# thunlp/ConvDR

Measured on AMD Instinct MI355X. Metric: passages encoded/sec + query x passage IP-scored/sec, 768-d, higher is better.
Workload: dtype bf16

## Files before the change

convdr_amd/csrc/encoder.hip:

```cpp
#include "gemm_launch.hpp"
#include "gemm_ln.hpp"
#include "cls_fold.hpp"

#include "../../include/convdr_hip.h"

namespace convdr {

struct EncBufs {
  int32_t* status;
  int32_t *tok_id, *tok_pos;
  bf16_t *X, *Q, *K, *Vt, *ctx, *Hm, *cls_b, *cls_ctx, *cls_x, *cls_x1;
  float *Y, *cls_y, *cls_f, *head_y;
  float* slab;
  int64_t ldt;
  size_t total;
};

constexpr int64_t SPLITK_MAX_ROWS = 42 * 128;
constexpr int SPLITK_MAX_SPLIT = 4;
static int64_t g_ffn2_splitk = 1;

static EncBufs enc_plan(const convdr_encoder_config* c, int64_t rows, int B, char* base) {
  EncBufs p;
  size_t o = 0;
// ... 226 lines not shown
}

extern "C" int convdr_encoder_forward(const convdr_encoder_config* cfg, const convdr_encoder_weights* w,
                                      const void* input_ids, int ids_are_int32, const int64_t* attention_mask, int B, int L,
                                      const int32_t* cu_seqlens, const int32_t* seq_lens, int64_t rows, int max_len,
                                      void* workspace, size_t workspace_bytes, float* out, convdr_stream_t stream) {
  hipStream_t st = (hipStream_t)stream;
  if (int e = check_config(cfg)) return e;
  CONVDR_REQUIRE(B > 0 && L > 0 && rows > 0 && rows % 8 == 0 && max_len > 0 && max_len <= L,
                 "convdr_encoder_forward: bad sizes B=%d L=%d rows=%lld max_len=%d", B, L, (long long)rows, max_len);
  const EncBufs p = enc_plan(cfg, rows, B, (char*)workspace);
  CONVDR_REQUIRE(workspace_bytes >= p.total, "convdr_encoder_forward: workspace too small (%zu < %zu)", workspace_bytes,
                 p.total);
  const int H = cfg->hidden;
  CONVDR_CHECK_HIP(hipMemset2DAsync(p.Vt + rows, p.ldt * 2, 0, (p.ldt - rows) * 2, H, st));
  CONVDR_CHECK_HIP(hipMemsetAsync(p.status, 0, 256, st));
  hipLaunchKernelGGL(k_seq_pack, dim3((B + 3) / 4), dim3(256), 0, st, input_ids, ids_are_int32, attention_mask, seq_lens, B, L, cu_seqlens,
                     cfg->kind, cfg->pad_idx, cfg->max_pos, cfg->vocab, p.tok_id, p.tok_pos, p.status);
  CONVDR_CHECK_LAUNCH("k_seq_pack");
  return encoder_forward_packed(cfg, w, p, cu_seqlens, seq_lens, rows, B, max_len, out, st);
}

extern "C" int convdr_encoder_forward_ragged(const convdr_encoder_config* cfg, const convdr_encoder_weights* w,
                                             const int32_t* tokens, int64_t n_tokens, const int32_t* tok_offsets, int B,
                                             const int32_t* cu_seqlens, const int32_t* seq_lens, int64_t rows, int max_len,
                                             void* workspace, size_t workspace_bytes, float* out, convdr_stream_t stream) {
  hipStream_t st = (hipStream_t)stream;
  if (int e = check_config(cfg)) return e;
  CONVDR_REQUIRE(B > 0 && n_tokens >= B && n_tokens <= INT32_MAX && rows > 0 && rows % 8 == 0 && rows >= n_tokens && max_len > 0 &&
                     max_len <= n_tokens,
                 "convdr_encoder_forward_ragged: bad sizes B=%d n_tokens=%lld rows=%lld max_len=%d", B, (long long)n_tokens,
                 (long long)rows, max_len);
  CONVDR_REQUIRE(tokens != nullptr && tok_offsets != nullptr, "convdr_encoder_forward_ragged: null tokens / tok_offsets");
  const EncBufs p = enc_plan(cfg, rows, B, (char*)workspace);
  CONVDR_REQUIRE(workspace_bytes >= p.total, "convdr_encoder_forward_ragged: workspace too small (%zu < %zu)", workspace_bytes,
                 p.total);
  const int H = cfg->hidden;
  CONVDR_CHECK_HIP(hipMemset2DAsync(p.Vt + rows, p.ldt * 2, 0, (p.ldt - rows) * 2, H, st));
  CONVDR_CHECK_HIP(hipMemsetAsync(p.status, 0, 256, st));
  hipLaunchKernelGGL(k_seq_pack_ragged, dim3((B + 3) / 4), dim3(256), 0, st, tokens, n_tokens, tok_offsets, seq_lens, B, cu_seqlens,
                     cfg->kind, cfg->pad_idx, cfg->max_pos, cfg->vocab, p.tok_id, p.tok_pos, p.status);
  CONVDR_CHECK_LAUNCH("k_seq_pack_ragged");
  return encoder_forward_packed(cfg, w, p, cu_seqlens, seq_lens, rows, B, max_len, out, st);
}

extern "C" int convdr_encoder_debug_layout(const convdr_encoder_config* cfg, int64_t rows, int B, int64_t* out) {
  const EncBufs p = enc_plan(cfg, rows, B, nullptr);
  const void* v[13] = {p.tok_id, p.tok_pos, p.X, p.Q, p.K, p.Vt, p.ctx, p.Hm, p.Y, p.cls_b, p.cls_y, p.cls_f, p.head_y};
  for (int i = 0; i < 13; ++i) out[i] = (int64_t)(size_t)v[i];
  out[13] = p.ldt;
  return 0;
}

namespace convdr {
static __global__ void __launch_bounds__(256) k_pack_kslice(const bf16_t* __restrict__ w, int n, int k, bf16_t* __restrict__ out) {
  const int64_t total = (int64_t)n * (k / 8);
  for (int64_t i = (int64_t)blockIdx.x * blockDim.x + threadIdx.x; i < total; i += (int64_t)gridDim.x * blockDim.x) {
    const int c = (int)(i & 3);
    const int64_t sr = i >> 2;
    const int r = (int)(sr % n), s = (int)(sr / n);
    *(uint4*)(out + i * 8) = *(const uint4*)(w + (int64_t)r * k + s * 32 + c * 8);
  }
}
}

extern "C" int convdr_pack_kslice(const void* w_bf16, int n, int k, void* out, convdr_stream_t stream) {
  CONVDR_REQUIRE(n > 0 && k > 0 && k % 32 == 0, "convdr_pack_kslice: bad shape %d x %d", n, k);
  const int64_t total = (int64_t)n * (k / 8);
  hipLaunchKernelGGL(k_pack_kslice, dim3((unsigned)(ceil_div64(total, 256) < 4096 ? ceil_div64(total, 256) : 4096)), dim3(256), 0,
                     (hipStream_t)stream, (const bf16_t*)w_bf16, n, k, (bf16_t*)out);
  CONVDR_CHECK_LAUNCH("k_pack_kslice");
  return 0;
}

extern "C" int convdr_set_option(const char* name, int64_t value) {
  if (strcmp(name, "fused_ln_min_rows") == 0) {
    g_fused_ln_min_rows = value;
    return 0;
  }
  if (strcmp(name, "hm_blocked") == 0) {
    g_hm_blocked = value;
    return 0;
  }
  if (strcmp(name, "cls_fold") == 0) {
    g_cls_fold = value;
    return 0;
  }
  if (strcmp(name, "cls_fold_min_rows") == 0) {
    g_cls_fold_min_rows = value;
    return 0;
  }
  if (strcmp(name, "gemm_tile_policy") == 0) {
    g_gemm_tile_policy = value;
    return 0;
  }
  if (strcmp(name, "attn_bwd_fused") == 0) {
    g_attn_bwd_fused = value;
    return 0;
  }
  if (strcmp(name, "embed_bwd_deterministic") == 0) {
    g_embed_bwd_det = value;
    return 0;
  }
  if (strcmp(name, "ip_fused_finish") == 0) {
    convdr::g_ip_fused_finish = value;
    return 0;
  }
  if (strcmp(name, "gelu_gp") == 0) {
    g_gelu_gp = value;
    return 0;
  }
  if (strcmp(name, "ffn2_splitk") == 0) {
    g_ffn2_splitk = value;
    return 0;
  }
  if (strcmp(name, "ln_rows") == 0) {
    g_ln_rows = value;
    return 0;
  }
  if (strcmp(name, "ln_bwd_rows") == 0) {
    g_ln_bwd_rows = value;
    return 0;
  }
  if (strcmp(name, "train_bwd_stop_layer") == 0) {
    g_train_bwd_stop_layer = value;
    return 0;
  }
  if (strcmp(name, "fused_ln_max_k") == 0) {
    g_fused_ln_max_k = value;
    return 0;
  }
  if (strcmp(name, "clock_probe") == 0) {
    g_clock_probe = (void*)(uintptr_t)value;
    g_clock_probe_next = 0;
    return 0;
  }
  if (strcmp(name, "clock_probe_slots") == 0) {
    g_clock_probe_slots = value > 0 ? value : 1;
    return 0;
  }
  if (strcmp(name, "attn_trace") == 0) {
    g_attn_trace = (void*)(uintptr_t)value;
    return 0;
  }
  if (strcmp(name, "gemm_trace_ln") == 0) {
    g_gemm_trace_ln = (void*)(uintptr_t)value;
    return 0;
  }
  if (strcmp(name, "gemm_trace") == 0) {
    g_gemm_trace = (void*)(uintptr_t)value;
    return 0;
  }
  set_error("convdr_set_option: unknown option %s", name);
  return -1;
}
```

convdr_amd/csrc/encoder_kernels.hpp:

```cpp
#pragma once
#include "../../include/convdr_hip.h"
#include "dropout.hpp"
#include "gemm_nt.hpp"

namespace convdr {

static __global__ void __launch_bounds__(256) k_seq_pack(const void* __restrict__ ids_v, int ids32,
                                                  const int64_t* __restrict__ mask, const int32_t* __restrict__ lens,
                                                  int B, int L, const int32_t* __restrict__ cu, int kind, int pad_idx,
                                                  int max_pos, int vocab, int32_t* __restrict__ tok_id,
                                                  int32_t* __restrict__ tok_pos, int32_t* __restrict__ status) {
  const int lane = threadIdx.x & 63;
  const int b = blockIdx.x * 4 + (threadIdx.x >> 6);
  if (b >= B) return;
  const int base = cu[b], end = cu[b + 1];
  const int64_t* ids = (const int64_t*)ids_v;
  const int32_t* ids_i = (const int32_t*)ids_v;
  const int len_b = lens[b];
  int kept = 0, nonpad = 0;
  int flags = 0;
  for (int l0 = 0; l0 < L; l0 += 64) {
    const int l = l0 + lane;
    const bool valid = l < L;
    int64_t id = valid ? (ids32 ? (int64_t)ids_i[(int64_t)b * L + l] : ids[(int64_t)b * L + l]) : (int64_t)pad_idx;
    const bool m = valid && (mask ? mask[(int64_t)b * L + l] != 0 : l < len_b);
    if (l == 0 && !m) flags |= CONVDR_ENC_STATUS_BAD_MASK;
    const bool np = valid && id != pad_idx;
    const unsigned long long bm = __ballot(m), bnp = __ballot(np);
    const unsigned long long lt = (1ull << lane) - 1ull;
    if (m) {
      if (id < 0 || id >= (int64_t)vocab) { flags |= CONVDR_ENC_STATUS_BAD_TOKEN; id = 0; }
      const int row = base + kept + __popcll(bm & lt);
      if (row < end) {
        int p = kind == 0 ? (np ? nonpad + __popcll(bnp & (lt | (1ull << lane))) + pad_idx : pad_idx) : l;
        p = p < max_pos ? p : max_pos - 1;
        tok_id[row] = (int)id;
        tok_pos[row] = p;
      }
    }
    kept += __popcll(bm);
    nonpad += __popcll(bnp);
  }
  if (kept != len_b) flags |= CONVDR_ENC_STATUS_BAD_LENS;
  if (__ballot(flags != 0) != 0ull) {
#pragma unroll
    for (int o = 32; o >= 1; o >>= 1) flags |= __shfl_xor(flags, o, 64);
    if (lane == 0) atomicOr(status, flags);
  }
  for (int r = base + kept + lane; r < end; r += 64) {
    tok_id[r] = -1;
    tok_pos[r] = 0;
  }
}

static __global__ void __launch_bounds__(256) k_seq_pack_ragged(const int32_t* __restrict__ tokens, int64_t n_tokens,
                                                         const int32_t* __restrict__ off, const int32_t* __restrict__ lens,
                                                         int B, const int32_t* __restrict__ cu, int kind, int pad_idx,
                                                         int max_pos, int vocab, int32_t* __restrict__ tok_id,
                                                         int32_t* __restrict__ tok_pos, int32_t* __restrict__ status) {
  const int lane = threadIdx.x & 63;
  const int b = blockIdx.x * 4 + (threadIdx.x >> 6);
  if (b >= B) return;
  const int base = cu[b], end = cu[b + 1];
  const int64_t o0 = off[b], o1 = off[b + 1];
  const int len_b = lens[b];
  const bool ok = o0 >= 0 && o0 <= o1 && o1 <= n_tokens && o1 - o0 == (int64_t)len_b && len_b >= 1 &&
                  (int64_t)len_b <= (int64_t)end - (int64_t)base;
  const int n = ok ? len_b : 0;
  int kept = 0, nonpad = 0;
  int flags = ok ? 0 : CONVDR_ENC_STATUS_BAD_LENS;
  for (int l0 = 0; l0 < n; l0 += 64) {
    const int l = l0 + lane;
    const bool m = l < n;
    int id = m ? tokens[o0 + l] : pad_idx;
    const bool np = m && id != pad_idx;
    const unsigned long long bm = __ballot(m), bnp = __ballot(np);
    const unsigned long long lt = (1ull << lane) - 1ull;
    if (m) {
      if (id < 0 || id >= vocab) { flags |= CONVDR_ENC_STATUS_BAD_TOKEN; id = 0; }
      const int row = base + kept + __popcll(bm & lt);
      int p = kind == 0 ? (np ? nonpad + __popcll(bnp & (lt | (1ull << lane))) + pad_idx : pad_idx) : l;
      p = p < max_pos ? p : max_pos - 1;
      tok_id[row] = id;
// ... 372 lines not shown
struct CTile {
  static constexpr int PASSES = (T::TL * T::TR * 2) / T::STAGE_BYTES;
  static constexpr int NTP = T::NT / PASSES;
  static constexpr int ROWS = T::TL / PASSES;
  static_assert(PASSES >= 1 && PASSES * NTP == T::NT, "a pass is a whole number of MFMA column blocks");
  static constexpr int HALF = ROWS / 2, HALF_BYTES = HALF * T::TR * 2;
  struct Base { uint32_t lo, hi; };
  __device__ static __forceinline__ Base contiguous(const char* sC) {
    static_assert(2 * HALF_BYTES <= T::STAGE_BYTES, "a parked pass must fit the idle stage");
    return Base{lds_off(sC), lds_off(sC) + HALF_BYTES};
  }
  static constexpr int CW = T::MT * 4;
  static constexpr int RW = NTP * 32;
  static constexpr int W_BYTES = RW * CW * 16;
  static constexpr int W_STORES = RW * CW / 64;
  static_assert(W_BYTES * T::WAVES <= 2 * HALF_BYTES && (64 % CW) == 0, "wave-local park must fit the pass image");
  __device__ static __forceinline__ uint32_t wave_base(Base sC, int wave) {
    constexpr int PER_HALF = HALF_BYTES / W_BYTES;
    return (wave >= PER_HALF ? sC.hi + (wave - PER_HALF) * W_BYTES : sC.lo + wave * W_BYTES);
  }
  __device__ static __forceinline__ void put_w(uint32_t wb, const WavePos<T>& w, int mt, int ntl, int g, uint2 o) {
    const int row = ntl * 32 + w.li;
    lds_write_b64_hidden(wb + row * (CW * 16) + (((mt * 4 + g) ^ (row & (CW - 1))) << 4) + w.hi * 8, (u32x2_t){o.x, o.y});
  }
  template <int C0, int CN>
  __device__ static __forceinline__ void store_w_part(bool nt, uint32_t wb, int lane, bf16_t* dst, int64_t ld, int64_t row_limit,
                                                      int64_t col_limit) {
    constexpr int RPI = 64 / CN, N_ST = RW / RPI;
    static_assert(64 % CN == 0 && N_ST % 4 == 0, "store_w_part geometry");
    const int r0 = lane / CN, c = C0 + (lane - r0 * CN);
    const int64_t nv = col_limit - c * 8;
#pragma unroll
    for (int i0 = 0; i0 < N_ST; i0 += 4) {
      u32x4_t v[4];
      auto at = [&](int i) {
        const int row = i * RPI + r0;
        return wb + row * (CW * 16) + ((c ^ (row & (CW - 1))) << 4);
      };
      lds_read4_b128_hidden(at(i0), at(i0 + 1), at(i0 + 2), at(i0 + 3), v[0], v[1], v[2], v[3]);
#pragma unroll
      for (int j = 0; j < 4; ++j) {
        const int row = (i0 + j) * RPI + r0;
        bf16_t* pr = dst + (int64_t)row * ld + c * 8;
        if (row < row_limit && nv > 0) {
          if (nv >= 8) {
            if (nt) store16<true>(pr, v[j]);
            else store16<false>(pr, v[j]);
          }
          else *(uint2*)pr = make_uint2(v[j].x, v[j].y);
        }
      }
    }
  }
  __device__ static __forceinline__ void store_w(bool nt, uint32_t wb, int lane, bf16_t* dst, int64_t ld, int64_t row_limit,
                                                 int64_t col_limit) {
    constexpr int RPI = 64 / CW;
    const int r0 = lane / CW, c = lane - r0 * CW;
    const int64_t nv = col_limit - c * 8;
    static_assert(W_STORES % 4 == 0, "lds_read4_b128_hidden reads four chunks");
#pragma unroll
    for (int i0 = 0; i0 < W_STORES; i0 += 4) {
      u32x4_t v[4];
      auto at = [&](int i) {
        const int row = i * RPI + r0;
        return wb + row * (CW * 16) + ((c ^ (row & (CW - 1))) << 4);
      };
      lds_read4_b128_hidden(at(i0), at(i0 + 1), at(i0 + 2), at(i0 + 3), v[0], v[1], v[2], v[3]);
#pragma unroll
      for (int j = 0; j < 4; ++j) {
        const int row = (i0 + j) * RPI + r0;
        bf16_t* pr = dst + (int64_t)row * ld + c * 8;
        if (row < row_limit && nv > 0) {
          if (nv >= 8) {
            if (nt) store16<true>(pr, v[j]);
            else store16<false>(pr, v[j]);
          }
          else *(uint2*)pr = make_uint2(v[j].x, v[j].y);
        }
      }
    }
  }
};

template <int EPI, class T>
static __global__ void __launch_bounds__(T::THREADS, 2) k_gemm(const GemmArgs a) {
  extern __shared__ __attribute__((aligned(16))) char smem[];
  using CT = CTile<T>;
  const WavePos<T> w;
  const int64_t ldw = a.ldw ? a.ldw : a.K, ldx = a.ldx ? a.ldx : a.K;
  int kbeg = 0, klen = a.K;
  if constexpr (EPI == EPI_SLAB_F32) {
    if (a.k_split_len) { kbeg = blockIdx.y * a.k_split_len; klen = a.k_split_len; }
  }
  const uint32_t ntiles = (uint32_t)a.tilesN * a.tilesT;
  const uint32_t xcd = blockIdx.x & 7u, q8 = ntiles >> 3, r8 = ntiles & 7u;
  const uint32_t chunk_base = xcd < r8 ? xcd * (q8 + 1) : r8 * (q8 + 1) + (xcd - r8) * q8;
  const uint32_t chunk_len = q8 + (xcd < r8 ? 1u : 0u);
  const uint32_t stride = (gridDim.x + 7u) >> 3;
  uint32_t idx = blockIdx.x >> 3;
  if (idx >= chunk_len) return;
  if (a.clock_probe && blockIdx.x == 0 && blockIdx.y == 0 && threadIdx.x == 0) {
    a.clock_probe[0] = __builtin_amdgcn_s_memtime();
    a.clock_probe[1] = __builtin_amdgcn_s_memrealtime();
  }

  struct Coord { int64_t t0; int n0; int swap; };
  auto decode = [&](uint32_t i) {
    const uint32_t logical = chunk_base + i;
    int tt = logical / a.tilesN, tn = logical - tt * a.tilesN;
    if (a.dbg_same_tile) { tt = 0; tn = 0; }
    Coord c;
    c.t0 = (int64_t)tt * T::TL;
    c.n0 = tn * T::TR;
    c.swap = false;
    if constexpr (EPI == EPI_QKV) c.swap = c.n0 + a.third0 * a.H >= 2 * a.H;
    return c;
  };
  auto tile_src = [&](const Coord& c) {
    return c.swap ? TileSrc<T>(a.X, ldx, a.rows, a.W, ldw, a.N, c.t0, c.n0, w)
                  : TileSrc<T>(a.W + kbeg, ldw, a.N, a.X + kbeg, ldx, a.rows, c.n0, c.t0, w);
  };

  constexpr bool R3 = T::WAVES == 8;
  R3Slots st{0, 0};
  auto sbias_of = [&](R3Slots s) { return (float*)(smem + (s.rs == 2 ? 0 : s.rs + 1) * T::R_BYTES); };
  auto tile_src_all = [&](const Coord& cc) {
    return cc.swap ? TileSrcAll<T>(a.X, ldx, a.rows, a.W, ldw, a.N, cc.t0, cc.n0, w)
                   : TileSrcAll<T>(a.W + kbeg, ldw, a.N, a.X + kbeg, ldx, a.rows, cc.n0, cc.t0, w);
  };
  float* sbias = R3 ? sbias_of(st) : (float*)(smem + T::SMEM_BYTES);
  int trace_tile = 0;
#ifdef CONVDR_ENABLE_TRACE
#define CONVDR_TRACE(ph)                                                                                       \
  if (a.trace && threadIdx.x == 0 && trace_tile < 64)                                                          \
    a.trace[((size_t)blockIdx.x * 64 + trace_tile) * 16 + (ph)] = __builtin_amdgcn_s_memtime();
#else
#define CONVDR_TRACE(ph)
#endif
  auto bias_slice = [&](const Coord& cc) {
    const int f = cc.n0 + (int)threadIdx.x;
    return (!cc.swap && a.bias && threadIdx.x < T::TR && f < a.N) ? a.bias[f] : 0.f;
  };
  Coord c = decode(idx);
  int buf = 0;
  bool landed = false;
  if (threadIdx.x < T::TR) sbias[threadIdx.x] = bias_slice(c);
  TileSrc<T> src = tile_src(c);
  TileSrcAll<T> src3 = tile_src_all(c);
  if constexpr (R3) gemm_r3_prologue<T>(src3, a.K, smem, w, st, false);
  else gemm_issue_stage<T>(src, 0, smem + buf * T::STAGE_BYTES, w);
  __syncthreads();
  for (;;) {
    const uint32_t next = idx + stride;
    const bool has_next = next < chunk_len;
    const Coord cn = has_next ? decode(next) : c;
    GemmAcc<T> acc;
    float bias_lane[T::NT];
    if (c.swap) {
      acc.zero();
#pragma unroll
      for (int nt = 0; nt < T::NT; ++nt) {
        const int f = c.n0 + w.l_index(nt);
        bias_lane[nt] = a.bias[f < a.N ? f : a.N - 1];
      }
    } else {
#pragma unroll
      for (int nt = 0; nt < T::NT; ++nt) bias_lane[nt] = 0.f;
#pragma unroll
      for (int mt = 0; mt < T::MT; ++mt) {
        u32x4_t bq[4];
        const uint32_t sb = lds_off(sbias);
        lds_read4_b128_hidden(sb + w.r_base(mt, 0) * 4, sb + w.r_base(mt, 1) * 4, sb + w.r_base(mt, 2) * 4,
                              sb + w.r_base(mt, 3) * 4, bq[0], bq[1], bq[2], bq[3]);
#pragma unroll
        for (int g = 0; g < 4; ++g)
#pragma unroll
          for (int nt = 0; nt < T::NT; ++nt) {
            acc.c[mt][nt][4 * g + 0] = __uint_as_float(bq[g].x); acc.c[mt][nt][4 * g + 1] = __uint_as_float(bq[g].y);
            acc.c[mt][nt][4 * g + 2] = __uint_as_float(bq[g].z); acc.c[mt][nt][4 * g + 3] = __uint_as_float(bq[g].w);
          }
      }
    }
    float bias_next = has_next ? bias_slice(cn) : 0.f;
    constexpr bool RES_PRE = EPI == EPI_RESID_F32 && T::WAVES == 4;
    uint2 res_pre[RES_PRE ? T::NT : 1][T::MT][4];
    if constexpr (RES_PRE) {
      if (a.Rf == nullptr) {
#pragma unroll
        for (int nt = 0; nt < T::NT; ++nt) {
          const int64_t t = c.t0 + w.l_index(nt);
          const int64_t tc = t < a.rows ? t : a.rows - 1;
#pragma unroll
          for (int mt = 0; mt < T::MT; ++mt)
#pragma unroll
            for (int g = 0; g < 4; ++g) {
              int f = c.n0 + w.r_base(mt, g);
              f = f < a.N ? f : a.N - 4;
              res_pre[nt][mt][g] = *(const uint2*)(a.R + tc * a.N + f);
            }
        }
      }
    }
    CONVDR_TRACE(0)
    int idle;
    if constexpr (R3) {
      st = gemm_nt_mainloop_r3<T>(src3, c.swap ? a.K : klen, smem, acc, w, st, true, true, landed || a.dbg_prelanded,
                                  (a.trace && trace_tile == 8) ? a.trace + ((size_t)blockIdx.x * 64 + 56) * 16 : nullptr);
      idle = 0;
      sbias = sbias_of(st);
    } else {
    idle = gemm_nt_mainloop<T>(src, c.swap ? a.K : klen, smem, acc, w, buf, true, landed,
                               (a.trace && trace_tile == 8) ? a.trace + ((size_t)blockIdx.x * 64 + 56) * 16 : nullptr);
    }
    landed = false;
    constexpr bool GP_PRE = EPI == EPI_MUL_GP;
    u32x4_t gp_pre[GP_PRE ? T::NT : 1][GP_PRE ? T::MT : 1][2];
    if constexpr (GP_PRE) {
      int tid_p = threadIdx.x;
      asm volatile("" : "+v"(tid_p));
      const WavePos<T> wp(tid_p);
      const int64_t rows32p = (a.rows + 31) & ~(int64_t)31;
#pragma unroll
      for (int nt = 0; nt < T::NT; ++nt) {
        const int64_t tb = c.t0 + (wp.wl * T::NT + nt) * 32;
        const int64_t tbc = tb < rows32p ? tb : 0;
#pragma unroll
        for (int mt = 0; mt < T::MT; ++mt) {
          const int f0 = c.n0 + wp.wr * T::MT * 32 + mt * 32;
          const int f0c = f0 < a.N ? f0 : 0;
          const bf16_t* blk = a.Gp + ((tbc >> 5) * (a.N >> 3) + (f0c >> 3)) * 256 + wp.li * 8;
#pragma unroll
          for (int j = 0; j < 2; ++j)
            gp_pre[nt][mt][j] = __builtin_nontemporal_load((const u32x4_t*)(blk + (int64_t)(2 * j + wp.hi) * 256));
        }
      }
    }
    asm volatile("" : "+v"(bias_next));
    if constexpr (RES_PRE) {
#pragma unroll
      for (int nt = 0; nt < T::NT; ++nt)
#pragma unroll
        for (int mt = 0; mt < T::MT; ++mt)
#pragma unroll
          for (int g = 0; g < 4; ++g) asm volatile("" : "+v"(res_pre[nt][mt][g].x), "+v"(res_pre[nt][mt][g].y));
    }
#pragma unroll
    for (int i = 0; i < T::NT; ++i) asm volatile("" : "+v"(bias_lane[i]));
    if (threadIdx.x < T::TR) sbias[threadIdx.x] = bias_next;
    CONVDR_TRACE(1)
    if (has_next) {
      if constexpr (R3) {
        src3 = tile_src_all(cn);
        gemm_r3_prologue<T>(src3, a.K, smem, w, st, false);
      } else {
        src = tile_src(cn);
        gemm_issue_stage<T>(src, 0, smem + idle * T::STAGE_BYTES, w);
      }
    }
    typename CT::Base sC;
    if constexpr (R3) {
      static_assert(T::R_BYTES >= CT::HALF_BYTES && 3 * T::R_BYTES + 2 * T::L_BYTES + (T::L_BYTES >= CT::HALF_BYTES ? 0 : CT::HALF_BYTES) <= 160 * 1024,
                    "parked pass: one dead R slot + one dead L slot (or the spare LDS behind the slots)");
      sC = typename CT::Base{lds_off(smem + (st.rs == 0 ? 2 : st.rs - 1) * T::R_BYTES),
                             T::L_BYTES >= CT::HALF_BYTES ? lds_off(smem + 3 * T::R_BYTES + (st.ls ^ 1) * T::L_BYTES)
                                                          : lds_off(smem + 3 * T::R_BYTES + 2 * T::L_BYTES)};
    } else {
      sC = CT::contiguous(smem + (idle ^ 1) * T::STAGE_BYTES);
    }
    int tid_e = threadIdx.x;
    asm volatile("" : "+v"(tid_e));
    const WavePos<T> we(tid_e);
    const int64_t t0 = c.t0;
    const int n0 = c.n0;

    if (a.dbg_skip_epi == 1) {
      float s = 0.f;
#pragma unroll
      for (int mt = 0; mt < T::MT; ++mt)
#pragma unroll
        for (int nt = 0; nt < T::NT; ++nt)
#pragma unroll
          for (int r = 0; r < 16; ++r) s += acc.c[mt][nt][r];
      if (s == 12345.678f) a.Cb[0] = f32_to_bf16(s);
    } else if (c.swap) {
      lds_barrier();
#pragma unroll
      for (int pass = 0; pass < CT::PASSES; ++pass) {
        const uint32_t wb = CT::wave_base(sC, we.wave);
#pragma unroll
        for (int ntl = 0; ntl < CT::NTP; ++ntl) {
          const int nt = pass * CT::NTP + ntl;
          const float bv = bias_lane[nt];
#pragma unroll
          for (int mt = 0; mt < T::MT; ++mt)
#pragma unroll
            for (int g = 0; g < 4; ++g) {
              const f32x16& v = acc.c[mt][nt];
              uint2 o;
              o.x = pack_bf16x2(v[4 * g + 0] + bv, v[4 * g + 1] + bv);
              o.y = pack_bf16x2(v[4 * g + 2] + bv, v[4 * g + 3] + bv);
              CT::put_w(wb, we, mt, ntl, g, o);
            }
        }
        if (pass == CT::PASSES - 1 && has_next) {
          lds_dma_wait_all();
          landed = true;
        }
        const int row0 = (we.wl * T::NT + pass * CT::NTP) * 32, col0 = we.wr * T::MT * 32;
        CT::store_w(a.nt_out != 0, wb, we.lane, a.Vt + (int64_t)(n0 + (a.third0 - 2) * a.H + row0) * a.ldt + t0 + col0, a.ldt,
                    a.N - n0 - row0, a.rows - t0 - col0);
      }
    } else if (EPI == EPI_GELU_BLK || (EPI == EPI_QKV && a.qk_blocked)) {
      lds_barrier();
      CONVDR_TRACE(2)
      const int64_t rows32 = (a.rows + 31) & ~(int64_t)31;
      bf16_t* dstm = a.Cb;
      int oct_w = a.N >> 3, f0 = n0;
      if constexpr (EPI == EPI_QKV) {
        const int na = n0 + a.third0 * a.H;
        dstm = na < a.H ? a.Qo : a.Ko;
        f0 = na < a.H ? na : na - a.H;
        oct_w = a.H >> 3;
      }
#pragma unroll
      for (int nt = 0; nt < T::NT; ++nt) {
        const int64_t tb = t0 + (we.wl * T::NT + nt) * 32;
        if (nt == T::NT - 1 && has_next) {
          lds_dma_wait_all();
          landed = true;
        }
        bf16_t* blk = dstm + ((tb >> 5) * oct_w + ((f0 + we.wr * T::MT * 32) >> 3)) * 256 + we.li * 8;
#pragma unroll
        for (int mt = 0; mt < T::MT; ++mt)
#pragma unroll
          for (int j = 0; j < 2; ++j) {
            uint2 o[2];
#pragma unroll
            for (int e = 0; e < 2; ++e) {
              const int g = 2 * j + e;
              const f32x16& v = acc.c[mt][nt];
              float y0 = v[4 * g + 0], y1 = v[4 * g + 1], y2 = v[4 * g + 2], y3 = v[4 * g + 3];
              if constexpr (EPI == EPI_GELU_BLK) { gelu_tail2(y0, y1); gelu_tail2(y2, y3); }
              o[e].x = pack_bf16x2(y0, y1);
              o[e].y = pack_bf16x2(y2, y3);
            }
            const auto sx = __builtin_amdgcn_permlane32_swap(o[0].x, o[1].x, false, false);
            const auto sy = __builtin_amdgcn_permlane32_swap(o[0].y, o[1].y, false, false);
            u32x4_t q;
            q.x = sx[0]; q.y = sy[0]; q.z = sx[1]; q.w = sy[1];
            if (tb < rows32 && n0 + we.wr * T::MT * 32 + mt * 32 < a.N)
              store16<NT_GEMM_BLK>(blk + (int64_t)(mt * 4 + 2 * j + we.hi) * 256, q);
          }
      }
      CONVDR_TRACE(6)
    } else {
      lds_barrier();
      CONVDR_TRACE(2)
// ... 425 lines not shown
```

convdr_amd/csrc/gemm_launch.hpp:

```cpp
#pragma once
#include <stdlib.h>

#include "encoder_kernels.hpp"

namespace convdr {

inline void* g_gemm_trace = nullptr;
inline void* g_gemm_trace_ln = nullptr;
inline void* g_attn_trace = nullptr;
inline void* g_clock_probe = nullptr;
inline int64_t g_clock_probe_slots = 1, g_clock_probe_next = 0;

template <int EPI, class T>
inline int launch_gemm_t(GemmArgs a, hipStream_t st, const char* prof_name) {
  static_assert(T::TR == T::TL || EPI != EPI_QKV, "square tiles: the QKV kernel swaps operand roles per tile");
  static DeviceOnce attr_done;
  if (attr_done.first()) {
    CONVDR_CHECK_HIP(
        hipFuncSetAttribute((const void*)k_gemm<EPI, T>, hipFuncAttributeMaxDynamicSharedMemorySize,
                            T::WAVES == 8 ? 160 * 1024 : T::SMEM_BYTES + T::TR * 4));
  }
#ifdef CONVDR_ENABLE_TRACE
  static const int dbg = getenv("CONVDR_DBG_SAME_TILE") ? atoi(getenv("CONVDR_DBG_SAME_TILE")) : 0;
  a.dbg_same_tile = dbg;
  static const int dbg_epi = getenv("CONVDR_DBG_SKIP_EPI") ? atoi(getenv("CONVDR_DBG_SKIP_EPI")) : 0;
  a.dbg_skip_epi = dbg_epi;
  static const int dbg_pre = getenv("CONVDR_DBG_PRELANDED") ? atoi(getenv("CONVDR_DBG_PRELANDED")) : 0;
  a.dbg_prelanded = dbg_pre;
  static const int trace_epi = getenv("CONVDR_TRACE_EPI") ? atoi(getenv("CONVDR_TRACE_EPI")) : (int)EPI_GELU_BF16;
#else
  constexpr int trace_epi = EPI_GELU_BF16;
#endif
  a.trace = (EPI == trace_epi) ? (unsigned long long*)g_gemm_trace : nullptr;
  a.clock_probe = nullptr;
  if (g_clock_probe && strcmp(prof_name, "gemm_ffn1") == 0) {
    a.clock_probe = (unsigned long long*)g_clock_probe + 4 * (g_clock_probe_next % g_clock_probe_slots);
    ++g_clock_probe_next;
  }
  a.nt_out = NT_CTILE && (int64_t)a.rows * a.N * 2 >= ((int64_t)128 << 20);
  a.tilesN = (a.N + T::TR - 1) / T::TR;
  a.tilesT = (int)ceil_div64(a.rows, T::TL);
  if (a.tilesT == 0) return 0;
  unsigned splits = 1;
  if (EPI == EPI_SLAB_F32 && a.k_split_len) {
    CONVDR_REQUIRE(a.k_split_len % GEMM_BK == 0 && a.K % a.k_split_len == 0, "gemm: bad split-K slice %d of %d",
                   a.k_split_len, a.K);
    splits = a.K / a.k_split_len;
  }
  ProfScope prof(prof_name, st);
  const int64_t slots = (int64_t)device_cu_count() * (T::SMEM_BYTES > 80 * 1024 ? 1 : 2);
  int64_t grid = (int64_t)a.tilesN * a.tilesT;
  if (splits == 1 && grid > slots) grid = slots;
  const size_t lds = T::WAVES == 8 ? 160 * 1024 : T::SMEM_BYTES + T::TR * 4;
  hipLaunchKernelGGL((k_gemm<EPI, T>), dim3((unsigned)grid, splits), dim3(T::THREADS), lds, st, a);
#ifdef CONVDR_ENABLE_TRACE
  static const int dbl = getenv("CONVDR_DBG_DOUBLE") ? atoi(getenv("CONVDR_DBG_DOUBLE")) : 0;
  if (dbl & (strcmp(prof_name, "gemm_dgrad") == 0 ? 2 : strncmp(prof_name, "gemm_", 5) == 0 && strcmp(prof_name, "gemm_cls") != 0 ? 1 : 0))
    hipLaunchKernelGGL((k_gemm<EPI, T>), dim3((unsigned)grid, splits), dim3(T::THREADS), lds, st, a);
#endif
  CONVDR_CHECK_LAUNCH("k_gemm");
  return 0;
}

inline int64_t g_gemm_tile_policy = 0;
inline int64_t g_attn_bwd_fused = 1;
inline int64_t g_embed_bwd_det = getenv("CONVDR_EMBED_BWD_DETERMINISTIC") ? atoi(getenv("CONVDR_EMBED_BWD_DETERMINISTIC")) : 0;
inline int64_t g_gelu_gp = 1;
inline int64_t g_ln_bwd_rows = 2;
inline int64_t g_train_bwd_stop_layer = -1;
struct TileCost { double step_us, epi_us; int per_cu; };
inline double gemm_tile_cost(int64_t tiles, int nk, const TileCost& c) {
  const int64_t slots = (int64_t)device_cu_count() * c.per_cu;
  return (double)ceil_div64(tiles, slots) * (nk * c.step_us + c.epi_us);
}
template <int EPI>
inline int launch_gemm(GemmArgs a, hipStream_t st, const char* prof_name) {
  CONVDR_REQUIRE(a.K % GEMM_BK == 0 && a.N % 4 == 0, "gemm: need K %% 64 == 0 and N %% 4 == 0 (K=%d N=%d)", a.K, a.N);
  if (EPI == EPI_QKV) CONVDR_REQUIRE(a.H % 128 == 0 && a.ldt % 8 == 0, "gemm: fused QKV needs hidden %% 128 == 0 (%d)", a.H);
  if (EPI == EPI_BF16 || EPI == EPI_GELU_BF16 || EPI == EPI_GELU_SAVE || EPI == EPI_GELU_BLK || EPI == EPI_GELU_GP || EPI == EPI_MUL_GP)
    CONVDR_REQUIRE(a.N % 8 == 0, "gemm: bf16 outputs are stored 16 bytes at a time, need N %% 8 == 0 (N=%d)", a.N);
  const bool fits = a.N % 256 == 0 && (EPI != EPI_QKV || a.H % 256 == 0);
  int splits = 1;
  if (EPI == EPI_SLAB_F32 && a.k_split_len) splits = a.K / a.k_split_len;
  const int64_t tiles256 = (int64_t)(a.N / 256) * ceil_div64(a.rows, 256) * splits;
  constexpr bool WIDE_OK = EPI == EPI_BF16 || EPI == EPI_RESID_F32 || EPI == EPI_GELU_SAVE || EPI == EPI_GELU_BF16 || EPI == EPI_F32 ||
                           EPI == EPI_GELU_GP || EPI == EPI_MUL_GP;
  int choice = (fits && tiles256 >= 192) ? 256 : 128;
  if (fits && g_gemm_tile_policy == 1) choice = 256;
  else if (fits && g_gemm_tile_policy == 3) choice = 128;
  else if (fits && WIDE_OK) {
    if (g_gemm_tile_policy == 2) choice = 192;
    else {
      const int nk = (EPI == EPI_SLAB_F32 && a.k_split_len ? a.k_split_len : a.K) / GEMM_BK;
      const int64_t tilesW = (int64_t)(a.N / 256) * ceil_div64(a.rows, 128) * splits;
      const int64_t tiles128 = (int64_t)(a.N / 128) * ceil_div64(a.rows, 128) * splits;
      static const TileCost c256{1.42, 4.0, 1}, cW{1.32, 2.5, 1}, c128{1.30, 2.0, 2};
      const double t256 = gemm_tile_cost(tiles256, nk, c256), tW = gemm_tile_cost(tilesW, nk, cW), t128 = gemm_tile_cost(tiles128, nk, c128);
      choice = (t256 <= tW && t256 <= t128) ? 256 : (tW <= t128 ? 192 : 128);
    }
  }
  if (fits && a.tile_hint == 256) choice = 256;
  if (choice == 256) return launch_gemm_t<EPI, Tile256>(a, st, prof_name);
  if constexpr (WIDE_OK) {
    if (choice == 192) return launch_gemm_t<EPI, TileWide>(a, st, prof_name);
  }
  return launch_gemm_t<EPI, Tile128>(a, st, prof_name);
}

}
```

convdr_amd/csrc/gemm_nt.hpp:

```cpp
#pragma once
#include "common.hpp"

namespace convdr {

constexpr int GEMM_BK = 64;

typedef const __attribute__((address_space(1))) void* gptr_t;
typedef __attribute__((address_space(3))) void* lptr_t;

__device__ __forceinline__ void glds16(const void* g, void* lds_wave_base) {
  __builtin_amdgcn_global_load_lds((gptr_t)g, (lptr_t)lds_wave_base, 16, 0, 0);
}
template <bool NT, class V>
__device__ __forceinline__ void store16(void* p, const V& v) {
  static_assert(sizeof(V) == 16, "16-byte store");
  typedef uint32_t raw4_t __attribute__((ext_vector_type(4)));
  if constexpr (NT) __builtin_nontemporal_store(__builtin_bit_cast(raw4_t, v), (raw4_t*)p);
  else *(V*)p = v;
}
constexpr bool NT_GEMM_BLK = true;
constexpr bool NT_CTILE = true;
constexpr bool NT_ATT = true;
constexpr bool NT_LN = true;
template <int AUX>
// ... 227 lines not shown
  char* sL = smem + 3 * T::R_BYTES;
  R3Issue<T>::template r<R_AUX>(src.R, 0, sR + s.rs * T::R_BYTES, w.wave);
  R3Issue<T>::l(src.L, 0, sL + s.ls * T::L_BYTES, w.wave);
  if (with_r1 && K > GEMM_BK) R3Issue<T>::template r<R_AUX>(src.R, 1, sR + (s.rs == 2 ? 0 : s.rs + 1) * T::R_BYTES, w.wave);
}
template <class T, bool F16 = false, int R_AUX = 0>
__device__ __forceinline__ R3Slots gemm_nt_mainloop_r3(const TileSrcAll<T>& src, int K, char* smem, GemmAcc<T>& acc,
                                                       const WavePos<T>& w, R3Slots st = R3Slots{0, 0},
                                                       bool prologue_in_flight = false, bool r1_deferred = false,
                                                       bool stage0_landed = false, unsigned long long* step_trace = nullptr) {
  constexpr int R_DPW = R3Issue<T>::R_DPW;
  const bool r_wave = R3Issue<T>::issues_r(w.wave);
  const int nk = K / GEMM_BK;
  const int sw = (w.lane >> 1) & 7;
  const int offR = (w.wr * T::MT * 32 + w.li) * 128;
  const int offL = (w.wl * T::NT * 32 + w.li) * 128;
  char* sR = smem;
  char* sL = smem + 3 * T::R_BYTES;
  if (!prologue_in_flight) gemm_r3_prologue<T, R_AUX>(src, K, smem, w, st, !r1_deferred);
  int rs = st.rs, ls = st.ls;
#ifdef CONVDR_ENABLE_TRACE
#define CONVDR_R3_STEP(i) \
  if (step_trace && kt == 6 + (i) / 6 && w.lane == 0) step_trace[w.wave * 8 + (i)] = __builtin_amdgcn_s_memtime();
#else
#define CONVDR_R3_STEP(i)
#endif
  for (int kt = 0; kt < nk; ++kt) {
    CONVDR_R3_STEP(6)
    CONVDR_R3_STEP(0)
    if (kt == 0 && (r1_deferred || stage0_landed)) {
      if (!stage0_landed) lds_dma_wait_all();
    } else if (kt + 1 < nk && r_wave) asm volatile("s_waitcnt vmcnt(%0)" ::"n"(R_DPW) : "memory");
    else lds_dma_wait_all();
    CONVDR_R3_STEP(1)
    lds_barrier();
    CONVDR_R3_STEP(2)
    const char* tR = sR + rs * T::R_BYTES + offR;
    const char* tL = sL + ls * T::L_BYTES + offL;
    bf16x8 fa[2][T::MT], fb[2][T::NT];
    auto load_frags = [&](int s, int set) {
      const int ch = ((2 * s + w.hi) ^ sw) * 16;
#pragma unroll
      for (int j = 0; j < T::NT; ++j) fb[set][j] = *(const bf16x8*)(tL + j * 32 * 128 + ch);
#pragma unroll
      for (int i = 0; i < T::MT; ++i) fa[set][i] = *(const bf16x8*)(tR + i * 32 * 128 + ch);
    };
    load_frags(0, 0);
    const bool issue_l = kt + 1 < nk, issue_r = kt + 2 < nk;
    char* l_dst = sL + (ls ^ 1) * T::L_BYTES;
    const int rnext = rs == 0 ? 2 : rs - 1;
    char* r_dst = sR + rnext * T::R_BYTES;
    __builtin_amdgcn_sched_barrier(0);
    if (r1_deferred && kt == 0 && issue_l) R3Issue<T>::template r<R_AUX>(src.R, 1, sR + (rs == 2 ? 0 : rs + 1) * T::R_BYTES, w.wave);
    if (issue_l) R3Issue<T>::l(src.L, kt + 1, l_dst, w.wave);
    CONVDR_R3_STEP(3)
#pragma unroll
    for (int s = 0; s < 4; ++s) {
      if (s + 1 < 4) load_frags(s + 1, (s + 1) & 1);
#pragma unroll
      for (int i = 0; i < T::MT; ++i)
#pragma unroll
        for (int j = 0; j < T::NT; ++j)
          acc.c[i][j] = mfma_32x32x16<F16>(fa[s & 1][i], fb[s & 1][j], acc.c[i][j]);
      if (s + 1 < 4) {
#pragma unroll
        for (int r = 0; r < T::MT + T::NT && r < T::MT * T::NT; ++r) {
          __builtin_amdgcn_sched_group_barrier(0x008, 1, 0);
          __builtin_amdgcn_sched_group_barrier(0x100, 1, 0);
        }
        __builtin_amdgcn_sched_group_barrier(0x100, T::MT + T::NT, 0);
        __builtin_amdgcn_sched_group_barrier(0x008, T::MT * T::NT, 0);
      }
      __builtin_amdgcn_sched_barrier(0);
    }
    CONVDR_R3_STEP(4)
    if (issue_r) R3Issue<T>::template r<R_AUX>(src.R, kt + 2, r_dst, w.wave);
    CONVDR_R3_STEP(5)
    rs = rs == 2 ? 0 : rs + 1;
    ls ^= 1;
  }
  return R3Slots{rs, ls};
}

template <class T>
__device__ __forceinline__ int gemm_nt_mainloop(const bf16_t* __restrict__ R, int64_t ldr, int64_t nR,
                                                const bf16_t* __restrict__ L, int64_t ldl, int64_t nL, int K,
                                                int64_t r0, int64_t l0, char* smem, GemmAcc<T>& acc,
                                                const WavePos<T>& w, int k_begin = 0) {
  const TileSrc<T> src(R + k_begin, ldr, nR, L + k_begin, ldl, nL, r0, l0, w);
  return gemm_nt_mainloop<T>(src, K, smem, acc, w);
}

}
```

Measured before the change: 45310.

## Use 16x16x32 MFMA mainloop and epilogue for blocked FFN1/QKV 256 tiles

Adds a GEMM variant built on 16x16x32 bf16 MFMA instructions. It has its own accumulator layout, an interleaved LDS read and MFMA schedule, and matching epilogues for the swapped (transposed V) and blocked outputs, using permlane16 swaps to assemble 16-byte stores. It is enabled by default for the blocked FFN1 (GELU) and blocked QKV GEMMs on 256x256 tiles, and can be switched off with an env var or a runtime option. The aim is better MFMA throughput or scheduling than the existing 32x32 instruction shape. In exchange it adds substantial new code paths with their own register pressure and layout risks.

```diff
diff --git a/convdr_amd/csrc/encoder.hip b/convdr_amd/csrc/encoder.hip
--- a/convdr_amd/csrc/encoder.hip
+++ b/convdr_amd/csrc/encoder.hip
@@ -332,6 +332,10 @@
     g_hm_blocked = value;
     return 0;
   }
+  if (strcmp(name, "mfma16") == 0) {
+    g_mfma16 = value;
+    return 0;
+  }
   if (strcmp(name, "cls_fold") == 0) {
     g_cls_fold = value;
     return 0;
diff --git a/convdr_amd/csrc/encoder_kernels.hpp b/convdr_amd/csrc/encoder_kernels.hpp
--- a/convdr_amd/csrc/encoder_kernels.hpp
+++ b/convdr_amd/csrc/encoder_kernels.hpp
@@ -1,4 +1,6 @@
 #pragma once
+#include <type_traits>
+
 #include "../../include/convdr_hip.h"
 #include "dropout.hpp"
 #include "gemm_nt.hpp"
@@ -537,10 +539,13 @@
   }
 };
 
-template <int EPI, class T>
+template <int EPI, class T, int MSHAPE = 0>
 static __global__ void __launch_bounds__(T::THREADS, 2) k_gemm(const GemmArgs a) {
   extern __shared__ __attribute__((aligned(16))) char smem[];
   using CT = CTile<T>;
+  constexpr bool M16 = MSHAPE == 1;
+  static_assert(MSHAPE == 0 || (M16 && (EPI == EPI_GELU_BLK || EPI == EPI_QKV) && T::WAVES == 8 && T::MT == 4 && T::NT == 2),
+                "16x16x32: blocked FFN1 / QKV on 256 x 256 tiles");
   const WavePos<T> w;
   const int64_t ldw = a.ldw ? a.ldw : a.K, ldx = a.ldx ? a.ldx : a.K;
   int kbeg = 0, klen = a.K;
@@ -609,9 +614,32 @@
     const uint32_t next = idx + stride;
     const bool has_next = next < chunk_len;
     const Coord cn = has_next ? decode(next) : c;
-    GemmAcc<T> acc;
-    float bias_lane[T::NT];
-    if (c.swap) {
+    std::conditional_t<M16, GemmAcc16<T>, GemmAcc<T>> acc;
+    float bias_lane[M16 ? 2 * T::NT : T::NT];
+    if constexpr (M16) {
+      if (c.swap) {
+        acc.zero();
+#pragma unroll
+        for (int j = 0; j < 2 * T::NT; ++j) {
+          const int f = c.n0 + w.wl * T::NT * 32 + 16 * j + (w.lane & 15);
+          bias_lane[j] = a.bias[f < a.N ? f : a.N - 1];
+        }
+      } else {
+#pragma unroll
+        for (int j = 0; j < 2 * T::NT; ++j) bias_lane[j] = 0.f;
+        const uint32_t sb = lds_off(sbias) + (w.wr * T::MT * 32 + 4 * (w.lane >> 4)) * 4;
+#pragma unroll
+        for (int i0 = 0; i0 < 2 * T::MT; i0 += 4) {
+          u32x4_t bq[4];
+          lds_read4_b128_hidden(sb + (i0 + 0) * 64, sb + (i0 + 1) * 64, sb + (i0 + 2) * 64, sb + (i0 + 3) * 64, bq[0], bq[1], bq[2], bq[3]);
+#pragma unroll
+          for (int g = 0; g < 4; ++g)
+#pragma unroll
+            for (int j = 0; j < 2 * T::NT; ++j)
+              acc.c[i0 + g][j] = (f32x4){__uint_as_float(bq[g].x), __uint_as_float(bq[g].y), __uint_as_float(bq[g].z), __uint_as_float(bq[g].w)};
+        }
+      }
+    } else if (c.swap) {
       acc.zero();
 #pragma unroll
       for (int nt = 0; nt < T::NT; ++nt) {
@@ -658,7 +686,11 @@
     }
     CONVDR_TRACE(0)
     int idle;
-    if constexpr (R3) {
+    if constexpr (M16) {
+      st = gemm_nt_mainloop_r3_m16<T>(src3, c.swap ? a.K : klen, smem, acc, w, st, true, true, landed || a.dbg_prelanded);
+      idle = 0;
+      sbias = sbias_of(st);
+    } else if constexpr (R3) {
       st = gemm_nt_mainloop_r3<T>(src3, c.swap ? a.K : klen, smem, acc, w, st, true, true, landed || a.dbg_prelanded,
                                   (a.trace && trace_tile == 8) ? a.trace + ((size_t)blockIdx.x * 64 + 56) * 16 : nullptr);
       idle = 0;
@@ -700,7 +732,7 @@
           for (int g = 0; g < 4; ++g) asm volatile("" : "+v"(res_pre[nt][mt][g].x), "+v"(res_pre[nt][mt][g].y));
     }
 #pragma unroll
-    for (int i = 0; i < T::NT; ++i) asm volatile("" : "+v"(bias_lane[i]));
+    for (int i = 0; i < (M16 ? 2 * T::NT : T::NT); ++i) asm volatile("" : "+v"(bias_lane[i]));
     if (threadIdx.x < T::TR) sbias[threadIdx.x] = bias_next;
     CONVDR_TRACE(1)
     if (has_next) {
@@ -728,6 +760,73 @@
     const int64_t t0 = c.t0;
     const int n0 = c.n0;
 
+    if constexpr (M16) {
+      const int q16 = we.lane >> 4, l16 = we.lane & 15;
+      lds_barrier();
+      if (c.swap) {
+#pragma unroll
+        for (int pass = 0; pass < CT::PASSES; ++pass) {
+          static_assert(CT::NTP == 1, "a pass is one 32-feature block: two 16-feature MFMA blocks");
+          const uint32_t wb = CT::wave_base(sC, we.wave);
+#pragma unroll
+          for (int jl = 0; jl < 2; ++jl) {
+            const int j = 2 * pass + jl;
+            const float bv = bias_lane[j];
+            const int row = jl * 16 + l16;
+#pragma unroll
+            for (int i = 0; i < 2 * T::MT; ++i) {
+              const f32x4& v = acc.c[i][j];
+              lds_write_b64_hidden(wb + row * (CT::CW * 16) + (((2 * i + (q16 >> 1)) ^ (row & (CT::CW - 1))) << 4) + (q16 & 1) * 8,
+                                   (u32x2_t){pack_bf16x2(v[0] + bv, v[1] + bv), pack_bf16x2(v[2] + bv, v[3] + bv)});
+            }
+          }
+          if (pass == CT::PASSES - 1 && has_next) {
+            lds_dma_wait_all();
+            landed = true;
+          }
+          const int row0 = (we.wl * T::NT + pass * CT::NTP) * 32, col0 = we.wr * T::MT * 32;
+          CT::store_w(a.nt_out != 0, wb, we.lane, a.Vt + (int64_t)(n0 + (a.third0 - 2) * a.H + row0) * a.ldt + t0 + col0, a.ldt,
+                      a.N - n0 - row0, a.rows - t0 - col0);
+        }
+      } else {
+        const int64_t rows32 = (a.rows + 31) & ~(int64_t)31;
+        bf16_t* dstm = a.Cb;
+        int oct_w = a.N >> 3, f0 = n0;
+        if constexpr (EPI == EPI_QKV) {
+          const int na = n0 + a.third0 * a.H;
+          dstm = na < a.H ? a.Qo : a.Ko;
+          f0 = na < a.H ? na : na - a.H;
+          oct_w = a.H >> 3;
+        }
+#pragma unroll
+        for (int g = 0; g < T::NT; ++g) {
+          const int64_t tb = t0 + (we.wl * T::NT + g) * 32;
+          if (g == T::NT - 1 && has_next) {
+            lds_dma_wait_all();
+            landed = true;
+          }
+          bf16_t* blk = dstm + ((tb >> 5) * oct_w + ((f0 + we.wr * T::MT * 32) >> 3) + (q16 >> 1)) * 256 + ((q16 & 1) * 16 + l16) * 8;
+#pragma unroll
+          for (int i = 0; i < 2 * T::MT; ++i) {
+            uint2 o[2];
+#pragma unroll
+            for (int e = 0; e < 2; ++e) {
+              const f32x4& v = acc.c[i][2 * g + e];
+              float y0 = v[0], y1 = v[1], y2 = v[2], y3 = v[3];
+              if constexpr (EPI == EPI_GELU_BLK) { gelu_tail2(y0, y1); gelu_tail2(y2, y3); }
+              o[e].x = pack_bf16x2(y0, y1);
+              o[e].y = pack_bf16x2(y2, y3);
+            }
+            const auto sx = __builtin_amdgcn_permlane16_swap(o[0].x, o[1].x, false, false);
+            const auto sy = __builtin_amdgcn_permlane16_swap(o[0].y, o[1].y, false, false);
+            u32x4_t q4;
+            q4.x = sx[0]; q4.y = sy[0]; q4.z = sx[1]; q4.w = sy[1];
+            if (tb < rows32 && n0 + we.wr * T::MT * 32 + i * 16 < a.N)
+              store16<NT_GEMM_BLK>(blk + (int64_t)(2 * i) * 256, q4);
+          }
+        }
+      }
+    } else
     if (a.dbg_skip_epi == 1) {
       float s = 0.f;
 #pragma unroll
diff --git a/convdr_amd/csrc/gemm_launch.hpp b/convdr_amd/csrc/gemm_launch.hpp
--- a/convdr_amd/csrc/gemm_launch.hpp
+++ b/convdr_amd/csrc/gemm_launch.hpp
@@ -11,13 +11,15 @@
 inline void* g_clock_probe = nullptr;
 inline int64_t g_clock_probe_slots = 1, g_clock_probe_next = 0;
 
-template <int EPI, class T>
+inline int64_t g_mfma16 = getenv("CONVDR_MFMA16") ? atoi(getenv("CONVDR_MFMA16")) : 1;
+
+template <int EPI, class T, int MSHAPE = 0>
 inline int launch_gemm_t(GemmArgs a, hipStream_t st, const char* prof_name) {
   static_assert(T::TR == T::TL || EPI != EPI_QKV, "square tiles: the QKV kernel swaps operand roles per tile");
   static DeviceOnce attr_done;
   if (attr_done.first()) {
     CONVDR_CHECK_HIP(
-        hipFuncSetAttribute((const void*)k_gemm<EPI, T>, hipFuncAttributeMaxDynamicSharedMemorySize,
+        hipFuncSetAttribute((const void*)k_gemm<EPI, T, MSHAPE>, hipFuncAttributeMaxDynamicSharedMemorySize,
                             T::WAVES == 8 ? 160 * 1024 : T::SMEM_BYTES + T::TR * 4));
   }
 #ifdef CONVDR_ENABLE_TRACE
@@ -52,11 +54,11 @@
   int64_t grid = (int64_t)a.tilesN * a.tilesT;
   if (splits == 1 && grid > slots) grid = slots;
   const size_t lds = T::WAVES == 8 ? 160 * 1024 : T::SMEM_BYTES + T::TR * 4;
-  hipLaunchKernelGGL((k_gemm<EPI, T>), dim3((unsigned)grid, splits), dim3(T::THREADS), lds, st, a);
+  hipLaunchKernelGGL((k_gemm<EPI, T, MSHAPE>), dim3((unsigned)grid, splits), dim3(T::THREADS), lds, st, a);
 #ifdef CONVDR_ENABLE_TRACE
   static const int dbl = getenv("CONVDR_DBG_DOUBLE") ? atoi(getenv("CONVDR_DBG_DOUBLE")) : 0;
   if (dbl & (strcmp(prof_name, "gemm_dgrad") == 0 ? 2 : strncmp(prof_name, "gemm_", 5) == 0 && strcmp(prof_name, "gemm_cls") != 0 ? 1 : 0))
-    hipLaunchKernelGGL((k_gemm<EPI, T>), dim3((unsigned)grid, splits), dim3(T::THREADS), lds, st, a);
+    hipLaunchKernelGGL((k_gemm<EPI, T, MSHAPE>), dim3((unsigned)grid, splits), dim3(T::THREADS), lds, st, a);
 #endif
   CONVDR_CHECK_LAUNCH("k_gemm");
   return 0;
@@ -100,6 +102,9 @@
     }
   }
   if (fits && a.tile_hint == 256) choice = 256;
+  if constexpr (EPI == EPI_GELU_BLK || EPI == EPI_QKV) {
+    if (choice == 256 && g_mfma16 != 0 && (EPI != EPI_QKV || a.qk_blocked)) return launch_gemm_t<EPI, Tile256, 1>(a, st, prof_name);
+  }
   if (choice == 256) return launch_gemm_t<EPI, Tile256>(a, st, prof_name);
   if constexpr (WIDE_OK) {
     if (choice == 192) return launch_gemm_t<EPI, TileWide>(a, st, prof_name);
diff --git a/convdr_amd/csrc/gemm_nt.hpp b/convdr_amd/csrc/gemm_nt.hpp
--- a/convdr_amd/csrc/gemm_nt.hpp
+++ b/convdr_amd/csrc/gemm_nt.hpp
@@ -333,6 +333,104 @@
   return R3Slots{rs, ls};
 }
 
+template <bool F16>
+__device__ __forceinline__ f32x4 mfma_16x16x32(const bf16x8& a, const bf16x8& b, const f32x4& c) {
+  if constexpr (F16)
+    return __builtin_amdgcn_mfma_f32_16x16x32_f16(__builtin_bit_cast(f16x8, a), __builtin_bit_cast(f16x8, b), c, 0, 0, 0);
+  else
+    return __builtin_amdgcn_mfma_f32_16x16x32_bf16(a, b, c, 0, 0, 0);
+}
+
+template <class T>
+struct GemmAcc16 {
+  static constexpr int MB = 2 * T::MT, NB = 2 * T::NT;
+  f32x4 c[MB][NB];
+  __device__ __forceinline__ void zero() {
+#pragma unroll
+    for (int i = 0; i < MB; ++i)
+#pragma unroll
+      for (int j = 0; j < NB; ++j) c[i][j] = (f32x4){0.f, 0.f, 0.f, 0.f};
+  }
+};
+
+template <class T, bool F16 = false, int R_AUX = 0>
+__device__ __forceinline__ R3Slots gemm_nt_mainloop_r3_m16(const TileSrcAll<T>& src, int K, char* smem, GemmAcc16<T>& acc,
+                                                           const WavePos<T>& w, R3Slots st = R3Slots{0, 0},
+                                                           bool prologue_in_flight = false, bool r1_deferred = false,
+                                                           bool stage0_landed = false) {
+  constexpr int MB = GemmAcc16<T>::MB, NB = GemmAcc16<T>::NB;
+  static_assert(MB == 8 && NB == 4, "the read schedule below is written for the 128 x 64 wave tile");
+  constexpr int R_DPW = R3Issue<T>::R_DPW;
+  const bool r_wave = R3Issue<T>::issues_r(w.wave);
+  const int nk = K / GEMM_BK;
+  const int sw = (w.lane >> 1) & 7;
+  const int q = w.lane >> 4;
+  const int offR = (w.wr * T::MT * 32 + (w.lane & 15)) * 128;
+  const int offL = (w.wl * T::NT * 32 + (w.lane & 15)) * 128;
+  const int ch0 = ((0 + q) ^ sw) * 16, ch1 = ((4 + q) ^ sw) * 16;
+  char* sR = smem;
+  char* sL = smem + 3 * T::R_BYTES;
+  if (!prologue_in_flight) gemm_r3_prologue<T, R_AUX>(src, K, smem, w, st, !r1_deferred);
+  int rs = st.rs, ls = st.ls;
+  for (int kt = 0; kt < nk; ++kt) {
+    if (kt == 0 && (r1_deferred || stage0_landed)) {
+      if (!stage0_landed) lds_dma_wait_all();
+    } else if (kt + 1 < nk && r_wave) asm volatile("s_waitcnt vmcnt(%0)" ::"n"(R_DPW) : "memory");
+    else lds_dma_wait_all();
+    lds_barrier();
+    const char* tR = sR + rs * T::R_BYTES + offR;
+    const char* tL = sL + ls * T::L_BYTES + offL;
+    bf16x8 fa[MB], fb[2][NB];
+    auto rdR = [&](int s2, int i) { return *(const bf16x8*)(tR + i * 16 * 128 + (s2 ? ch1 : ch0)); };
+    auto rdL = [&](int s2, int j) { return *(const bf16x8*)(tL + j * 16 * 128 + (s2 ? ch1 : ch0)); };
+#pragma unroll
+    for (int j = 0; j < NB; ++j) fb[0][j] = rdL(0, j);
+    fa[0] = rdR(0, 0);
+    fa[1] = rdR(0, 1);
+    const bool issue_l = kt + 1 < nk, issue_r = kt + 2 < nk;
+    char* l_dst = sL + (ls ^ 1) * T::L_BYTES;
+    const int rnext = rs == 0 ? 2 : rs - 1;
+    char* r_dst = sR + rnext * T::R_BYTES;
+    __builtin_amdgcn_sched_barrier(0);
+    if (r1_deferred && kt == 0 && issue_l) R3Issue<T>::template r<R_AUX>(src.R, 1, sR + (rs == 2 ? 0 : rs + 1) * T::R_BYTES, w.wave);
+    if (issue_l) R3Issue<T>::l(src.L, kt + 1, l_dst, w.wave);
+#pragma unroll
+    for (int i = 0; i < MB; ++i) {
+#pragma unroll
+      for (int j = 0; j < NB; ++j) {
+        acc.c[i][j] = mfma_16x16x32<F16>(fa[i], fb[0][j], acc.c[i][j]);
+        const int m = NB * i + j;
+        if (m < 6) fa[m + 2] = rdR(0, m + 2);
+        else if (m < 10) fb[1][m - 6] = rdL(1, m - 6);
+        else if (m < 12) fa[m - 10] = rdR(1, m - 10);
+      }
+      if (i >= 3) fa[i - 1] = rdR(1, i - 1);
+    }
+    fa[MB - 1] = rdR(1, MB - 1);
+#pragma unroll
+    for (int r = 0; r < 12; ++r) {
+      __builtin_amdgcn_sched_group_barrier(0x008, 1, 0);
+      __builtin_amdgcn_sched_group_barrier(0x100, 1, 0);
+    }
+#pragma unroll
+    for (int r = 0; r < 5; ++r) {
+      __builtin_amdgcn_sched_group_barrier(0x008, 4, 0);
+      __builtin_amdgcn_sched_group_barrier(0x100, 1, 0);
+    }
+    __builtin_amdgcn_sched_group_barrier(0x100, 1, 0);
+    __builtin_amdgcn_sched_barrier(0);
+#pragma unroll
+    for (int i = 0; i < MB; ++i)
+#pragma unroll
+      for (int j = 0; j < NB; ++j) acc.c[i][j] = mfma_16x16x32<F16>(fa[i], fb[1][j], acc.c[i][j]);
+    __builtin_amdgcn_sched_barrier(0);
+    if (issue_r) R3Issue<T>::template r<R_AUX>(src.R, kt + 2, r_dst, w.wave);
+    rs = rs == 2 ? 0 : rs + 1;
+    ls ^= 1;
+  }
+  return R3Slots{rs, ls};
+}
+
 template <class T>
 __device__ __forceinline__ int gemm_nt_mainloop(const bf16_t* __restrict__ R, int64_t ldr, int64_t nR,
                                                 const bf16_t* __restrict__ L, int64_t ldl, int64_t nL, int K,
```

After: 46740 (median of 6 runs). 3.1% higher.
